# zaphB/freecad.optics_design_workbench

Hardware: AMD Instinct MI355X
Metric: Monte-Carlo rays/sec (whole node), lensesAndMirrors.FCStd (higher is better)
Workload: dtype f64; 1 GPU; benchmark/lensesAndMirrors.FCStd, 1e+08 Monte-Carlo rays per step per GPU (BASELINE configs[2]), Gaussian point source sigma=1e-2, Philox4x32-10 seed 0x0D15EA5E; record_hit_rows=True, histogram=1024x1024 u64, parallelism=ray-index sharding x1, one RCCL reduce

## Files before the change

### freecad/optics_design_workbench_amd/csrc/odw_build.h

```cpp
#pragma once

#include <algorithm>
#include <cmath>
#include <cstdint>
#include <cstdio>
#include <cstring>
#include <limits>
#include <map>
#include <string>
#include <utility>
#include <vector>

namespace {

using namespace odw;

struct HostScene {
  std::vector<double> prim_f64;
  std::vector<int32_t> prim_i32;
  std::vector<int32_t> cond;
  std::vector<double> prim_hdr;
  std::vector<char> dead;
  std::vector<double> group_f64, group_gdir;
  std::vector<int32_t> group_i32;
// ... 1107 lines not shown
    for (std::vector<int>& set : inside[p]) {
      std::sort(set.begin(), set.end());
      set.erase(std::unique(set.begin(), set.end()), set.end());
    }
    std::sort(inside[p].begin(), inside[p].end());
  }
  for (int p = 0; p < n; ++p) {
    box_of[p] = p;
    for (int q = 0; q < p; ++q)
      if (!dead[q] && !dead[p] && hs.prim_i32[4 * q + 1] == hs.prim_i32[4 * p + 1] && inside[q] == inside[p]) {
        box_of[p] = q;
        box_shared[q] = 1;
        break;
      }
  }
}

constexpr int kSpecImageLimits = 4;
constexpr size_t kSpecArgBytes = 4096 - 512;

struct SpecLayout {
  int n = 0, ng = 0, size = 0;
  int gf = 0, gd = 0, gi = 0;
  std::vector<int> frame, par, box, der;
  std::vector<int> box_of, box_shared;
  std::vector<int> dc;
  bool fits(size_t params_bytes) const { return ((params_bytes + 7) & ~(size_t)7) + 8 + (size_t)size * 8 <= kSpecArgBytes; }
};

inline int spec_derived_count(int type) {
  switch (type) {
    case ODW_PRIM_BOX: return 3;
    case ODW_PRIM_CYLINDER: case ODW_PRIM_CONE: case ODW_PRIM_PARABOLOID: case ODW_PRIM_TORUS: return 4;
    case ODW_PRIM_CONICOID: case ODW_PRIM_ASPHERE: return 3;
    default: return 0;
  }
}

inline SpecLayout spec_image_layout(const HostScene& hs, const int32_t* disp_kind = nullptr) {
  SpecLayout L;
  const int n = L.n = hs.n_prims, ng = L.ng = hs.n_groups;
  spec_box_sharing(hs, L.box_of, L.box_shared);
  int at = kSpecImageLimits;
  L.gf = at; at += 4 * ng;
  L.gd = at; at += 3 * ng;
  L.gi = at; at += 2 * ng;
  L.frame.assign(n, 0); L.par.assign(n, 0); L.box.assign(n, -1); L.der.assign(n, -1);
  for (int p = 0; p < n; ++p) {
    const bool faces = (((hs.prim_i32[4 * p + 2]) >> ODW_FACEMASK_SHIFT) & 0xff) != 0;
    L.frame[p] = at; at += __builtin_popcount(xf_stored(xf_pattern(&hs.prim_f64[16 * (size_t)p])));
    L.par[p] = at; at += hs.prim_i32[4 * p] == ODW_PRIM_ASPHERE ? 4 + ODW_ASPH_ROW : 4;
    if (faces && L.box_of[p] == p) { L.box[p] = at; at += 6; }
    const int nd = faces ? spec_derived_count(hs.prim_i32[4 * p]) : 0;
    if (nd) { L.der[p] = at; at += nd; }
  }
  if (disp_kind) {
    L.dc.assign(std::max(1, ng), -1);
    for (int g = 0; g < ng; ++g)
      if (disp_kind[g]) { L.dc[g] = at; at += ODW_DISP_COEFS; }
  }
  L.size = at;
  return L;
}

inline void box_centre_half(double lo, double hi, double& c, double& h) {
#pragma clang fp contract(off)
  c = 0.5 * lo + 0.5 * hi;
  h = std::max(hi - c, c - lo);
  if (!(h >= 0.0)) h = 0.0;
  while (c - h > lo || c + h < hi) h = std::nextafter(h, INFINITY);
}

inline void spec_image_build(const HostScene& hs, const DeviceLimits& lim, const SpecLayout& L, double* img,
                             const double* disp_coef = nullptr) {
#pragma clang fp contract(off)
  const double tol = lim.dist_tol;
  std::fill(img, img + L.size, 0.0);
  if (disp_coef)
    for (int g = 0; g < (int)L.dc.size() && g < L.ng; ++g)
      if (L.dc[g] >= 0) std::memcpy(&img[L.dc[g]], disp_coef + ODW_DISP_COEFS * g, ODW_DISP_COEFS * sizeof(double));
  img[0] = tol;
  img[1] = lim.max_ray_length + tol;
  img[2] = 2.0 * tol;
  for (int g = 0; g < L.ng; ++g) {
    for (int k = 0; k < 4; ++k) img[L.gf + 4 * g + k] = hs.group_f64[4 * (size_t)g + k];
    for (int k = 0; k < 3; ++k) img[L.gd + 3 * g + k] = hs.group_gdir[3 * (size_t)g + k];
    std::memcpy(&img[L.gi + 2 * g], &hs.group_i32[4 * (size_t)g], 4 * sizeof(int32_t));
  }
  for (int p = 0; p < L.n; ++p) {
    const double* pf = &hs.prim_f64[16 * (size_t)p];
    const double* par = pf + 12;
    const unsigned stored = xf_stored(xf_pattern(pf));
    int at = L.frame[p];
    for (int i = 0; i < 12; ++i)
      if ((stored >> i) & 1u) img[at++] = pf[i];
    for (int k = 0; k < 4; ++k) img[L.par[p] + k] = par[k];
    if (hs.prim_i32[4 * p] == ODW_PRIM_ASPHERE)
      for (int k = 0; k < ODW_ASPH_ROW; ++k) img[L.par[p] + 4 + k] = hs.asph[ODW_ASPH_ROW * (size_t)p + k];
    if (L.box[p] >= 0) {
      const double* b = &hs.prim_hdr[8 * (size_t)p];
      for (int a = 0; a < 3; ++a) box_centre_half(b[a], b[3 + a], img[L.box[p] + a], img[L.box[p] + 3 + a]);
    }
    if (L.der[p] < 0) continue;
    double* d = img + L.der[p];
    const int type = hs.prim_i32[4 * p];
    if (type == ODW_PRIM_BOX) {
      for (int a = 0; a < 3; ++a) d[a] = par[a] + tol;
    } else if (type == ODW_PRIM_TORUS) {
      const double R1 = par[0], R2 = par[1];
      d[0] = std::fma(R1 + R2, 1.0000001, 1e-9);
// ... 165 lines not shown
```

### freecad/optics_design_workbench_amd/csrc/odw_capi.hip

```cpp
#include <hip/hip_runtime.h>
#include <hipcub/hipcub.hpp>

#include <algorithm>
#include <atomic>
#include <array>
#include <cmath>
#include <cstdio>
#include <cstdlib>
#include <cstring>
#include <condition_variable>
#include <functional>
#include <mutex>
#include <new>
#include <thread>
#include <string>
#include <utility>
#include <vector>

#include "odw_kernels.hip"
#include "odw_grid.hip"
#include "odw_mesh.hip"
#include "odw_build.h"

using namespace odw;
// ... 1320 lines not shown
int odw_spec_image(const odw_scene_desc* scene, const odw_limits* limits, double* image, uint64_t image_capacity,
                   uint64_t* image_size, int32_t* offsets, uint64_t offsets_capacity, double* boxes,
                   int32_t* in_arguments) {
  if (!scene || !limits) return fail(nullptr, ODW_ERR_INVALID, "odw_spec_image: null argument");
  if (!(limits->dist_tol > 0) || !(limits->max_ray_length > 0)) return fail(nullptr, ODW_ERR_INVALID, "odw_spec_image: limits out of range");
  HostScene tmp;
  std::string refusal;
  int rc = scene_host_tables(scene, tmp, refusal);
  if (rc) return fail(nullptr, rc, refusal);
  std::vector<Box> built;
  compute_boxes(tmp, limits->dist_tol, built);
  const std::string why = spec_ineligible(tmp);
  if (!why.empty()) return fail(nullptr, ODW_ERR_UNSUPPORTED, "odw_spec_image: " + why);
  const SpecLayout L = spec_image_layout(tmp);
  if (image_size) *image_size = (uint64_t)L.size;
  if (in_arguments) *in_arguments = L.fits(sizeof(TraceParams)) ? 1 : 0;
  if (image) {
    if (image_capacity < (uint64_t)L.size) return fail(nullptr, ODW_ERR_CAPACITY, "odw_spec_image: image_capacity too small");
    DeviceLimits lim;
    lim.max_ray_length = limits->max_ray_length;
    lim.dist_tol = limits->dist_tol;
    lim.power_tol = limits->power_tol;
    lim.max_intersections = limits->max_intersections;
    spec_image_build(tmp, lim, L, image);
  }
  if (boxes)
    for (int p = 0; p < L.n; ++p) std::memcpy(boxes + 6 * (size_t)p, &tmp.prim_hdr[8 * (size_t)p], 6 * sizeof(double));
  if (offsets) {
    if (offsets_capacity < 3 + 5 * (uint64_t)L.n) return fail(nullptr, ODW_ERR_CAPACITY, "odw_spec_image: offsets_capacity too small");
    offsets[0] = L.gf; offsets[1] = L.gd; offsets[2] = L.gi;
    for (int p = 0; p < L.n; ++p) {
      int32_t* o = offsets + 3 + 5 * p;
      o[0] = L.frame[p]; o[1] = L.par[p]; o[2] = L.box[p]; o[3] = L.der[p]; o[4] = L.box_of[p];
    }
  }
  return ODW_OK;
}

int odw_build_check(const odw_scene_desc* scene, const odw_limits* limits, int32_t* structure, uint64_t* sizes) {
  if (!scene || !limits) return fail(nullptr, ODW_ERR_INVALID, "odw_build_check: null argument");
  if (!(limits->dist_tol > 0) || limits->max_intersections < 0 || !(limits->max_ray_length > 0))
    return fail(nullptr, ODW_ERR_INVALID, "odw_build_check: limits out of range");
  int flat_limit = kBvhThreshold;
  if (const char* e = getenv("ODW_BVH_THRESHOLD")) flat_limit = atoi(e);
  HostScene tmp;
  SceneAccel A;
  std::string err;
// ... 492 lines not shown
  if (!ctx->have_limits) return fail(ctx, ODW_ERR_NO_SCENE, "odw_upload_scene_batch before odw_set_limits (the boxes carry the tolerance)");
  if (ctx->fresnel_on)
    return fail(ctx, ODW_ERR_UNSUPPORTED, "odw_upload_scene_batch: a batch with a Fresnel mode set (per-scene Fresnel modes are out of scope; "
                                          "odw_set_fresnel with n_groups = 0 clears it)");
  HIPCHK(ctx, hipSetDevice(ctx->device));
  ctx->batch_n = 0;
  ctx->batch_traced = 0;
  ctx->batch_rows_ok = false;
  ctx->phb_valid = ctx->phb_projected = false;
  int rc = odw_upload_scene(ctx, &scenes[0]);
  if (rc) return rc;
  if ((rc = build_bvh(ctx))) return rc;
  const bool compiled = ctx->compile_mode != ODW_COMPILE_OFF && spec_ineligible(ctx->hs).empty();
  const bool rare_compiled = flat_but_for_rare_quadrics(ctx->hs, ctx->flat_limit) && compiled && ctx->compile_mode == ODW_COMPILE_STRUCTURE;
  if ((ctx->P.scene.n_nodes || ctx->P.grid.nx > 0) && !rare_compiled)
    return fail(ctx, ODW_ERR_UNSUPPORTED, "odw_upload_scene_batch: batches are traced by the flat kernels (analytic scenes of up to 64 primitives; "
                                          "with paraboloids, ellipsoids, conicoids or aspheres: by the compiled one, ODW_COMPILE_STRUCTURE)");
  const bool eligible = spec_ineligible(ctx->hs).empty();
  const std::string text0 = eligible ? spec_text(ctx->hs, ctx->n_samplers) : std::string();
  const SpecLayout L0 = eligible ? spec_image_layout(ctx->hs) : SpecLayout();
  bool images = eligible;
  const size_t n = (size_t)ctx->P.scene.n_prims;
  const size_t o_hdr = 16 * n, o_gf = o_hdr + 8 * n, o_gd = o_gf + ODW_MAX_GROUPS * 4, o_img = o_gd + ODW_MAX_GROUPS * 3,
               stride = o_img + (size_t)L0.size;
  std::vector<double> blocks(stride * (size_t)n_scenes, 0.0);
  for (int k = 0; k < n_scenes; ++k) {
    HostScene tmp;
    std::string why;
    if ((rc = scene_host_tables(&scenes[k], tmp, why))) return fail(ctx, rc, why);
    if (!same_structure(ctx->hs, tmp, why))
      return fail(ctx, ODW_ERR_UNSUPPORTED, "odw_upload_scene_batch: scene " + std::to_string(k) + " differs from scene 0 in structure (" + why + ")");
    std::vector<Box> boxes;
    compute_boxes(tmp, ctx->P.lim.dist_tol, boxes);
    if (eligible && spec_text(tmp, ctx->n_samplers) != text0) {
      if (compiled)
        return fail(ctx, ODW_ERR_UNSUPPORTED, "odw_upload_scene_batch: scene " + std::to_string(k) + " differs from scene 0 in the structure a "
                                              "compiled kernel is built from (which frame entries are 0 / +1 / -1, shared boxes)");
      images = false;
    }
    double* b = blocks.data() + stride * (size_t)k;
    if (images) spec_image_build(tmp, ctx->P.lim, L0, b + o_img);
    std::memcpy(b, tmp.prim_f64.data(), 16 * n * sizeof(double));
    std::memcpy(b + o_hdr, tmp.prim_hdr.data(), 8 * n * sizeof(double));
    for (size_t p = 0; p < n; ++p) {
      int32_t w[4];
      std::memcpy(w, b + o_hdr + 8 * p + 6, sizeof w);
      w[2] &= ~ODW_FLAG_ISOLATED;
      std::memcpy(b + o_hdr + 8 * p + 6, w, sizeof w);
    }
    std::memcpy(b + o_gf, tmp.group_f64.data(), ODW_MAX_GROUPS * 4 * sizeof(double));
    std::memcpy(b + o_gd, tmp.group_gdir.data(), ODW_MAX_GROUPS * 3 * sizeof(double));
  }
  if ((rc = upload(ctx, ctx->batch_values, blocks.data(), blocks.size() * sizeof(double)))) return rc;
  std::vector<int32_t> pi = ctx->hs.prim_i32;
  for (size_t p = 0; p < n; ++p) pi[4 * p + 2] &= ~ODW_FLAG_ISOLATED;
  if (n && (rc = upload(ctx, ctx->prim_i32, pi.data(), pi.size() * sizeof(int32_t)))) return rc;
  if ((rc = upload_done(ctx))) return rc;
  ctx->hs.prim_i32 = pi;
  ctx->batch_n = n_scenes;
  ctx->batch_prims = n;
  ctx->batch_stride = stride;
  ctx->batch_img_off = images ? o_img : 0;
  ctx->batch_spec_text = compiled ? text0 : std::string();
  return ODW_OK;
// ... 624 lines not shown
```

### freecad/optics_design_workbench_amd/csrc/odw_kernels.hip

```cpp
#include "odw_device.h"

namespace odw {

#define ODW_CONST __attribute__((address_space(4)))
typedef const double ODW_CONST* cf64;
typedef const int32_t ODW_CONST* ci32;
typedef const uint64_t ODW_CONST* cu64;
template <class T>
__device__ __forceinline__ const T ODW_CONST* as_const(const T* p) {
  return (const T ODW_CONST*)(uintptr_t)p;
}
template <class T>
__device__ __forceinline__ const T* opaque(const T* p) {
  asm volatile("" : "+s"(p));
  return p;
}
typedef const DeviceSource ODW_CONST* csource;
typedef const DeviceDetector ODW_CONST* cdetector;

__device__ __forceinline__ double frcp(double x) {
  double r = __builtin_amdgcn_rcp(x);
  r = fma(fma(-x, r, 1.0), r, r);
  r = fma(fma(-x, r, 1.0), r, r);
  return r;
// ... 114 lines not shown
  return mk(m[0] * p.x + m[1] * p.y + m[2] * p.z + m[3],
            m[4] * p.x + m[5] * p.y + m[6] * p.z + m[7],
            m[8] * p.x + m[9] * p.y + m[10] * p.z + m[11]);
}
template <class P>
__device__ __forceinline__ d3 xf_vec(P m, d3 v) {
  return mk(m[0] * v.x + m[1] * v.y + m[2] * v.z, m[4] * v.x + m[5] * v.y + m[6] * v.z,
            m[8] * v.x + m[9] * v.y + m[10] * v.z);
}
template <class P>
__device__ __forceinline__ d3 xf_vec_t(P m, d3 v) {
  return mk(m[0] * v.x + m[4] * v.y + m[8] * v.z, m[1] * v.x + m[5] * v.y + m[9] * v.z,
            m[2] * v.x + m[6] * v.y + m[10] * v.z);
}

struct NoSpec {
  static constexpr bool enabled = false;
  static constexpr int N = 0;
  static constexpr int NG = 0;
  static constexpr unsigned long long xf(int) { return 0xfffull; }
  static constexpr int type(int) { return 0; }
  static constexpr int gtype(int) { return 0; }
  static constexpr int cond(int) { return 0; }
  static constexpr bool isolated() { return true; }
};
struct NoSource {
  static constexpr bool enabled = false;
  static constexpr bool single_row = false, phi_guide = false, finite_focal = false;
  static constexpr unsigned long long xf = 0xfffull;
};
template <unsigned long long XF, int IA, int IB, int IC, int IT, class P>
__device__ __forceinline__ double xf_comb(P m, double a, double b, double c) {
  double acc = 0.0;
  bool have = false;
#define ODW_XF_TERM(I, V)                                                                            \
  if constexpr (((XF >> (I)) & 1ull) != 0) {                                                         \
    if constexpr (((XF >> (12 + (I))) & 1ull) != 0) acc = have ? acc + (V) : (V);                    \
    else if constexpr (((XF >> (24 + (I))) & 1ull) != 0) acc = have ? acc - (V) : -(V);              \
    else acc = have ? fma(m[I], (V), acc) : m[I] * (V);                                              \
    have = true;                                                                                     \
  }
  ODW_XF_TERM(IB, b)
  ODW_XF_TERM(IA, a)
  ODW_XF_TERM(IC, c)
#undef ODW_XF_TERM
  if constexpr (IT >= 0) {
    if constexpr (((XF >> (IT < 0 ? 0 : IT)) & 1ull) != 0) acc = have ? m[IT < 0 ? 0 : IT] + acc : m[IT < 0 ? 0 : IT];
// ... 845 lines not shown
  a = fma(b.cz, inv.z, -oi.z); w = fabs(inv.z);
  lo = fmax(lo, fma(-b.hz, w, a)); hi = fmin(hi, fma(b.hz, w, a));
  return hi >= fmax(lo, 0.0) && lo < tmax;
}
template <class SPEC>
constexpr bool spec_live(int pi) { return !SPEC::dead(pi) && (SPEC::seq() || ((SPEC::umask() >> SPEC::group(pi)) & 1) != 0); }
template <class SPEC>
constexpr bool spec_own_box(int pi) { return spec_live<SPEC>(pi) && SPEC::box_of(pi) == pi; }
template <class SPEC>
constexpr int spec_next_box(int from) {
  for (int p = from; p < SPEC::N; ++p)
    if (spec_own_box<SPEC>(p)) return p;
  return -1;
}
template <class SPEC, int PI>
__device__ __forceinline__ SpecBox spec_box(const SceneView& sv) {
  static_assert(PI >= 0 && PI < SPEC::N, "box block of a primitive the scene does not have");
  static_assert(SPEC::box(PI) >= 0 && SPEC::box(PI) <= SPEC::IMG - 6, "box block outside the value image");
  cf64 bx = sv.img + SPEC::box(PI);
  return SpecBox{bx[0], bx[1], bx[2], bx[3], bx[4], bx[5]};
}

template <class SPEC, int PI>
__device__ __forceinline__ void spec_prim(const SceneView& sv, Query& q, d3 oi, d3 inv, int skip_solid, int only_solid,
                                          uint64_t mask, bool* boxhit, SpecBox& pending) {
  constexpr int flags = SPEC::flags(PI);
  if constexpr (spec_live<SPEC>(PI)) {
    [[maybe_unused]] const SpecBox own = pending;
    if constexpr (SPEC::box_of(PI) == PI && spec_next_box<SPEC>(PI + 1) >= 0) pending = spec_box<SPEC, spec_next_box<SPEC>(PI + 1)>(sv);
    if ((!SPEC::seq() || ((mask >> SPEC::group(PI)) & 1)) && (flags >> ODW_SOLID_SHIFT) != skip_solid &&
        (!SPEC::isolated() || only_solid < 0 || (flags >> ODW_SOLID_SHIFT) == only_solid)) {
      bool in_box;
      if constexpr (SPEC::box_of(PI) != PI) {
        in_box = boxhit[SPEC::box_of(PI)];
      } else {
        const double cut = q.cut;
        in_box = ray_box_centred(own, oi, inv, cut);
#if ODW_DOUBLE == 1
        in_box = in_box & ray_box_centred(own, mk(opq(oi.x), oi.y, oi.z), inv, cut);
#endif
      }
      boxhit[PI] = in_box;
      if (in_box)
        intersect_prim<SPEC::rare(), SPEC, PI>(sv, q, PI, SPEC::type(PI), SPEC::group(PI), flags, SPEC::cond_word(PI));
#if ODW_DOUBLE == 3 || ODW_DOUBLE == 4 || ODW_DOUBLE == 12
      if (in_box && SPEC::type(PI) == (ODW_DOUBLE == 3 ? ODW_PRIM_CYLINDER : (ODW_DOUBLE == 4 ? ODW_PRIM_BOX : ODW_PRIM_SPHERE))) {
        Query q2 = q;
        q2.start.x = opq(q.start.x);
        intersect_prim<SPEC::rare(), SPEC, PI>(sv, q2, PI, SPEC::type(PI), SPEC::group(PI), flags, SPEC::cond_word(PI));
        q.any = q2.any; q.oth = q2.oth;
      }
#endif
    } else if constexpr (SPEC::box_of(PI) == PI) {
      boxhit[PI] = SPEC::box_shared(PI) ? ray_box_centred(own, oi, inv, q.cut) : false;
    }
  }
}
template <class T, T... I> struct IndexList {};
template <class SPEC, int... PI>
__device__ __forceinline__ void spec_prims(const SceneView& sv, Query& q, d3 oi, d3 inv, int skip_solid, int only_solid,
                                           uint64_t mask, IndexList<int, PI...>) {
  bool boxhit[sizeof...(PI)] = {};
  SpecBox pending = {};
  if constexpr (spec_next_box<SPEC>(0) >= 0) pending = spec_box<SPEC, spec_next_box<SPEC>(0)>(sv);
  (spec_prim<SPEC, PI>(sv, q, oi, inv, skip_solid, only_solid, mask, boxhit, pending), ...);
}

template <bool BVH, class SPEC = NoSpec, bool ASPH = false>
__device__ __forceinline__ int nearest(const DeviceScene& sc, const SceneView& sv,
                                       const DeviceLimits& lim, d3 start, d3 dn, int medium,
                                       uint64_t mask, double& t_hit, int& face,
                                       int* __restrict__ stack, int skip_solid, int only_solid = -1) {
  Query q;
  q.start = start; q.dn = dn;
  if constexpr (SPEC::enabled) { q.tol = sv.lim[0]; q.tmax = sv.lim[1]; }
  else { q.tol = lim.dist_tol; q.tmax = lim.max_ray_length + lim.dist_tol; }
  q.medium = medium;
  q.in_medium = __ballot(medium >= 0) != 0ull;
  q.cut = q.tmax;
  q.any.t = INFINITY; q.any.prim = 0x7fffffff; q.any.face = 0x7fffffff;
  q.oth = q.any;
#if ODW_DOUBLE == 9
  d3 inv = mk(frcp1(dn.x), frcp1(dn.y), frcp1(dn.z));
  d3 oi = mk(start.x * inv.x, start.y * inv.y, start.z * inv.z);
  {
    const d3 dn2 = mk(opq(dn.x), opq(dn.y), opq(dn.z));
    const d3 inv2 = mk(frcp1(dn2.x), frcp1(dn2.y), frcp1(dn2.z));
    const d3 oi2 = mk(start.x * inv2.x, start.y * inv2.y, start.z * inv2.z);
    inv = inv2.x == inv.x ? inv : inv2;
    oi = oi2.y == oi.y ? oi : oi2;
  }
#else
  const d3 inv = mk(frcp1(dn.x), frcp1(dn.y), frcp1(dn.z));
  const d3 oi = mk(start.x * inv.x, start.y * inv.y, start.z * inv.z);
#endif
  if constexpr (SPEC::enabled) {
    spec_prims<SPEC>(sv, q, oi, inv, skip_solid, only_solid, mask, __make_integer_seq<IndexList, int, SPEC::N>{});
  } else if (!BVH) {
    const bool per_lane_mask = sc.seq_enabled != 0;
    const uint64_t umask = sc.all_mask & ~sc.ignore_mask;
    for (int p = 0; p < sc.n_prims; ++p) {
      cf64 hdr = sv.prim_hdr + 8 * p;
      ci32 hi = (ci32)(hdr + 6);
      const int type = hi[0], g = hi[1], flags = hi[2], cond_word = hi[3];
      if (per_lane_mask) {
        if (!((mask >> g) & 1)) continue;
      } else {
        if (!((umask >> g) & 1)) continue;
      }
      if ((flags >> ODW_SOLID_SHIFT) == skip_solid) continue;
      if (only_solid >= 0 && (flags >> ODW_SOLID_SHIFT) != only_solid) continue;
      const double cut = fmin(q.tmax, q.any.t + 2.0 * q.tol);
      if (!ray_box(hdr, oi, inv, cut)) continue;
      intersect_prim<0>(sv, q, p, type, g, flags, cond_word);
    }
  } else {
    typedef const float ODW_CONST* cf32;
    typedef float vf4 __attribute__((ext_vector_type(4)));
    typedef int vi4 __attribute__((ext_vector_type(4)));
    cf32 nodes = (cf32)(uintptr_t)sc.bvh_nodes;
    ci32 bvh_prims = as_const(sc.bvh_prims);
    const float ofx = (float)start.x, ofy = (float)start.y, ofz = (float)start.z;
    const float ivx = (float)inv.x, ivy = (float)inv.y, ivz = (float)inv.z;
    int sp = 0;
    int cur = 0;
    int pend = -1;
    for (;;) {
      for (;;) {
        const unsigned long long looking = __ballot(cur >= 0 && pend == -1);
        if (!(cur >= 0 && (pend == -1 || looking != 0ull))) break;
        cf32 nd = nodes + (size_t)cur * 16;
        const vf4 a0 = *reinterpret_cast<const vf4 ODW_CONST*>(nd);
        const vf4 a1 = *reinterpret_cast<const vf4 ODW_CONST*>(nd + 4);
        const vf4 a2 = *reinterpret_cast<const vf4 ODW_CONST*>(nd + 8);
        const vi4 lk = *reinterpret_cast<const vi4 ODW_CONST*>(nd + 12);
        const float cutf = (float)fmin(q.tmax, q.any.t + 2.0 * q.tol) * 1.00001f + 1e-3f;
        float tn0, tf0, tn1, tf1;
        {
          const float x0 = (a0.x - ofx) * ivx, x1 = (a0.w - ofx) * ivx;
// ... 406 lines not shown
  ray_uniforms(ray, seed, up, ut);
  sample_source(src, up, ut, t, phi);
  make_ray(src, t, phi, r.point, r.dir);
  r.power = src->power;
  return r;
}

template <class SRC>
__device__ __forceinline__ RayInit generate_ray_spec(csource src, uint64_t ray, uint64_t seed) {
  RayInit r;
  double up, ut, t, phi;
  ray_uniforms(ray, seed, up, ut);
  sample_source<true, SRC::phi_guide, SRC::single_row>(src, up, ut, t, phi);
  make_ray<SRC>(src, t, phi, r.point, r.dir);
  r.power = src->power;
  return r;
}

template <class SRC>
__device__ __noinline__ RayInit generate_ray_spec_call(csource src, uint64_t ray, uint64_t seed) {
  return generate_ray_spec<SRC>(src, ray, seed);
}

constexpr bool can_be_medium(int gtype) {
  return gtype != ODW_OPT_MIRROR && gtype != ODW_OPT_ABSORBER && gtype != ODW_OPT_VACUUM;
}
template <class SPEC, int G = 0>
constexpr int spec_media() {
  if constexpr (G >= SPEC::NG) return 0;
  else return (can_be_medium(SPEC::gtype(G)) ? 1 : 0) + spec_media<SPEC, G + 1>();
}
template <class SPEC, int K, int G = 0>
__device__ __forceinline__ double spec_medium_word(cf64 group_f64, int medium, double v) {
  if constexpr (G < SPEC::NG) {
    v = spec_medium_word<SPEC, K, G + 1>(group_f64, medium, v);
    if constexpr (can_be_medium(SPEC::gtype(G))) v = medium == G ? group_f64[4 * G + K] : v;
  }
  return v;
}
template <class SPEC, int K>
__device__ __forceinline__ double medium_word(cf64 group_f64, int medium) {
  if constexpr (SPEC::enabled && spec_media<SPEC>() <= 8) return spec_medium_word<SPEC, K>(group_f64, medium, 0.0);
  else return group_f64[4 * medium + K];
}

template <class SPEC, int G = 0>
__device__ __forceinline__ double spec_chroma_index(cf64 group_f64, int g, double wl, double v) {
  if constexpr (G < SPEC::NG) {
    v = spec_chroma_index<SPEC, G + 1>(group_f64, g, wl, v);
// ... 124 lines not shown
                                         int& skip, int& only, bool& alive, const DeviceChroma* C, double wl) {
  constexpr int flags = SPEC::flags(PI), g = SPEC::group(PI);
  const PackedFrame<SPEC::xf(PI)> pf{sv.img + SPEC::frame(PI)};
  cf64 par = sv.img + SPEC::par(PI);
  d3 n = face_normal<SPEC::rare()>(SPEC::type(PI), par, face, xf_point_nz<SPEC::xf(PI)>(pf, point), par + 4);
  if constexpr ((flags & ODW_FLAG_FLIP_NORMAL) != 0) n = n * -1.0;
  n = xf_vec_t_nz<SPEC::xf(PI)>(pf, n);
#if ODW_DOUBLE == 6
  {
    d3 n2 = face_normal<SPEC::rare()>(SPEC::type(PI), par, face, xf_point_nz<SPEC::xf(PI)>(pf, mk(opq(point.x), point.y, point.z)), par + 4);
    if constexpr ((flags & ODW_FLAG_FLIP_NORMAL) != 0) n2 = n2 * -1.0;
    n2 = xf_vec_t_nz<SPEC::xf(PI)>(pf, n2);
    n = n2.x == n.x ? n : n2;
  }
#endif
  const bool entering = dot(dir, n) < 0;
  if (entering) n = n * -1.0;
  constexpr int fmode = spec_fresnel<SPEC, FRESNEL>(g);
  interact<false, STOCH, LEAN, POWER, SPEC, CHROMA, FRESNEL>(P, group_f64, group_i32, group_gdir, g, SPEC::gtype(g), SPEC::record(g), n, entering, ray,
                               nint, cnt, hit_state, win, point, dir, power, medium, seq, alive, C, wl, fmode);
  const double out = entering ? -dot(dir, n) : dot(dir, n);
  if constexpr ((flags & ODW_FLAG_CONVEX) != 0) skip = out > 0 ? (flags >> ODW_SOLID_SHIFT) : -1;
  else skip = -1;
  if constexpr ((flags & ODW_FLAG_ISOLATED) != 0) only = out < 0 ? (flags >> ODW_SOLID_SHIFT) : -1;
  else only = -1;
}
template <bool STOCH, bool LEAN, bool POWER, class SPEC, bool CHROMA, bool FRESNEL, int... PI>
__device__ __forceinline__ void spec_hits(const TraceParams& P, const SceneView& sv, cf64 group_f64, ci32 group_i32,
                                          cf64 group_gdir, int prim, int face, uint64_t ray, int nint, uint32_t* cnt,
                                          uint32_t* hit_state, uint32_t* win, d3 point, d3& dir, double& power, int& medium, int& seq,
                                          int& skip, int& only, bool& alive, const DeviceChroma* C, double wl, IndexList<int, PI...>) {
  (void)((prim == PI ? (spec_hit<STOCH, LEAN, POWER, SPEC, CHROMA, FRESNEL, PI>(P, sv, group_f64, group_i32, group_gdir, face, ray, nint, cnt, hit_state, win,
                                                  point, dir, power, medium, seq, skip, only, alive, C, wl), true)
                     : false) || ...);
}

__device__ __forceinline__ void close_hit_block(const TraceParams& P, volatile uint32_t* hit_state, uint32_t next_scene) {
  if (!P.out.hit_block) {
    if (P.batch.n_scenes && __lane_id() == 0) hit_state[3] = next_scene;
    return;
  }
  odw_hit* hits = P.out.hits;
  unsigned long long* hit_count = P.out.hit_count;
  if (P.batch.n_scenes) {
    const uint32_t cur = __builtin_amdgcn_readfirstlane(hit_state[3]);
    hits += (size_t)cur * P.out.hit_capacity;
    hit_count += 4 * cur;
// ... 172 lines not shown
          }
#endif
        }
        seq = 0; nint = 0; medium = -1; skip = -1; only = -1;
        alive = true;
        if constexpr (CHROMA)
          wl = C->ray_wl ? C->ray_wl[i] : spectrum_wavelength(C->spec_tab, C->spec_n, C->spec_mode, P.first_ray + i, P.seed);
      }
      next += take;
      if (take == 0 && idle == ~0ull) break;
    }
    ODW_FTIME(0);
    if (alive) {
      if (nint >= lim.max_intersections) {
        ODW_COUNT(ODW_CNT_CAPPED);
        alive = false;
      } else {
      ++nint;
      uint64_t mask = sc.all_mask;
      if (sc.seq_enabled) mask = (seq < sc.seq_len) ? seq_mask[seq] : 0ull;
      mask &= ~sc.ignore_mask;
      double t_hit;
      int face;
      const int prim = nearest<BVH, SPEC, ASPH>(sc, sv, lim, point, dir, medium, mask, t_hit, face,
                                          bvh_stack + threadIdx.x, skip, BVH ? -1 : only);
      if (!BVH && prim < 0 && only >= 0) {
        only = -1;
        --nint;
        continue;
      }
      ODW_FTIME(1);
      if (SEG)
        record_segment(P.out.segs, P.out.seg_capacity, P.out.seg_count, P.first_ray + i, nint - 1, medium, point,
                       point + dir * (prim < 0 ? lim.max_ray_length : t_hit), power);
      if (prim < 0) {
        ODW_COUNT(ODW_CNT_ESCAPED);
        alive = false;
      } else {
      point = point + dir * t_hit;
      if (!LEAN && medium >= 0) {
        const double L = medium_word<SPEC, 2>(group_f64, medium);
        if (L == 0) power = 0;
        else if (L < INFINITY) power = exp(-t_hit / L);
      }
      uint32_t* cnt = cnt_lds + threadIdx.x;
      uint32_t* hit_state = hit_lds + (threadIdx.x >> 6) * 4;
      if constexpr (SPEC::enabled) {
        spec_hits<STOCH, LEAN, POWER, SPEC, CHROMA, FRESNEL>(P, sv, group_f64, group_i32, group_gdir, prim, face, P.first_ray + i, nint, cnt, hit_state,
// ... 350 lines not shown
```

### freecad/optics_design_workbench_amd/csrc/odw_spec.hip

```cpp
#include <dlfcn.h>
#include <hip/hiprtc.h>
#include <sys/stat.h>
#include <unistd.h>

#include <atomic>
#include <chrono>
#include <map>
#include <memory>
#include <mutex>
#include <thread>

#if !defined(__HIP_DEVICE_COMPILE__)
__asm__(
    ".pushsection .rodata\n"
    ".global odw_src_kernels\nodw_src_kernels:\n.incbin \"odw_kernels.hip\"\n.byte 0\n"
    ".global odw_src_device\nodw_src_device:\n.incbin \"odw_device.h\"\n.byte 0\n"
    ".global odw_src_trace\nodw_src_trace:\n.incbin \"../../../include/odw_trace.h\"\n.byte 0\n"
    ".popsection\n");
#endif
extern "C" const char odw_src_kernels[], odw_src_device[], odw_src_trace[];

namespace {

int spec_max_prims() {
// ... 100 lines not shown
    xf[p] = xf_pattern(&hs.prim_f64[16 * (size_t)p]);
  }
  const SpecLayout L = spec_image_layout(hs, disp_kind);
  const std::vector<int>&box_of = L.box_of, &box_shared = L.box_shared;
  std::vector<int> gtype(std::max(1, ng)), grec(std::max(1, ng));
  for (int g = 0; g < ng; ++g) { gtype[g] = hs.group_i32[4 * g]; grec[g] = hs.group_i32[4 * g + 1]; }
  auto fi = [](int v) { return std::to_string(v); };
  auto fu = [](unsigned long long v) { char b[32]; snprintf(b, sizeof b, "0x%llxull", v); return std::string(b); };
  std::string s;
  s += "struct Spec {\n  static constexpr bool enabled = true;\n";
  s += "  static constexpr int N = " + std::to_string(n) + ";\n";
  s += "  static constexpr int NG = " + std::to_string(ng) + ";\n";
  s += table("int", "type", n, type.data(), fi) + table("int", "group", n, group.data(), fi) +
       table("int", "flags", n, flags.data(), fi) + table("int", "cond_word", n, condw.data(), fi) +
       table("bool", "dead", n, dead.data(), fi) + table("int", "box_of", n, box_of.data(), fi) +
       table("bool", "box_shared", n, box_shared.data(), fi) +
       table("int", "cond", (int)hs.cond.size(), hs.cond.data(), fi) +
       table("unsigned long long", "xf", n, xf.data(), fu) + table("int", "gtype", ng, gtype.data(), fi) +
       table("bool", "record", ng, grec.data(), fi);
  int rare = 0;
  for (int p = 0; p < n; ++p) rare |= (type[p] == ODW_PRIM_PARABOLOID ? 1 : 0) | (type[p] == ODW_PRIM_ELLIPSOID ? 2 : 0) | (type[p] == ODW_PRIM_CONICOID ? 4 : 0) |
                                      (type[p] == ODW_PRIM_ASPHERE ? 8 : 0);
  s += "  static constexpr int rare() { return " + std::to_string(rare) + "; }\n";
  s += "  static constexpr bool isolated() { return false; }\n";
  s += "  static constexpr int IMG = " + std::to_string(L.size) + ";\n";
  s += std::string("  static constexpr bool img_fits = ") + (L.fits(sizeof(TraceParams) + (disp_kind ? sizeof(DeviceChroma) : 0)) ? "true" : "false") + ";\n";
  if (disp_kind) {
    std::vector<int> kinds(std::max(1, ng), 0);
    for (int g = 0; g < ng; ++g) kinds[g] = disp_kind[g];
    s += "  static constexpr bool chroma() { return true; }\n";
    s += table("int", "disp", ng, kinds.data(), fi) + table("int", "dc", ng, L.dc.data(), fi);
  }
  bool any_fresnel = false;
  for (int g = 0; fresnel && g < ng; ++g) any_fresnel |= fresnel[g] != 0;
  if (any_fresnel) {
    std::vector<int> modes(std::max(1, ng), 0);
    for (int g = 0; g < ng; ++g) modes[g] = fresnel[g];
    s += table("int", "fresnel", ng, modes.data(), fi);
  }
  s += "  static constexpr int gf = " + std::to_string(L.gf) + ", gd = " + std::to_string(L.gd) + ", gi = " + std::to_string(L.gi) + ";\n";
  s += table("int", "frame", n, L.frame.data(), fi) + table("int", "par", n, L.par.data(), fi) +
       table("int", "box", n, L.box.data(), fi) + table("int", "der", n, L.der.data(), fi);
  s += "  static constexpr int cond_off(int i) { return cond_word(i) & 0xffffff; }\n"
       "  static constexpr int cond_cnt(int i) { return (cond_word(i) >> 24) & 0xff; }\n";
  s += "  static constexpr unsigned long long umask() { return " + fu(hs.all_mask & ~hs.ignore_mask) + "; }\n";
  s += std::string("  static constexpr bool seq() { return ") + (hs.seq_enabled ? "true" : "false") + "; }\n";
  s += "};\n";
  s += std::string("#define ODW_SPEC_LEAN ") + (hs.lean ? "true" : "false") + "\n";
// ... 269 lines not shown
  ctx->spec_fn = it->second.fn;
  ctx->spec_lean = ctx->hs.lean;
  ctx->spec_stoch = ctx->n_samplers > 0;
  return ODW_OK;
}

void spec_note_launch(odw_ctx* ctx, uint64_t n_rays) {
  if (ctx->compile_mode != ODW_COMPILE_AUTO || !ctx->spec_pending) return;
  SpecGlobal& G = spec_global();
  std::lock_guard<std::mutex> lock(G.mu);
  uint64_t& rays = G.rays[ctx->spec_key];
  rays += n_rays;
  if (rays < ctx->spec_hot_rays) return;
  auto jt = G.jobs.find(ctx->spec_key);
  if (jt == G.jobs.end() || jt->second->done.load()) ctx->spec_dirty = true;
}

int spec_launch(odw_ctx* ctx, unsigned grid, hipFunction_t fn, bool batch, const DeviceChroma* chroma = nullptr) {
  const SpecLayout& L = chroma ? ctx->spec_chroma_layout : ctx->spec_layout;
  if (L.n != ctx->hs.n_prims || L.size < kSpecImageLimits) return fail(ctx, ODW_ERR_DEVICE, "compiled kernel without its value image");
  constexpr size_t tail = (sizeof(TraceParams) + 7) & ~(size_t)7;
  const bool resident = !batch && L.fits(sizeof(TraceParams) + (chroma ? sizeof(DeviceChroma) : 0));
  std::vector<double>& img = ctx->spec_image_now;
  img.resize((size_t)L.size);
  spec_image_build(ctx->hs, ctx->P.lim, L, img.data(), chroma ? ctx->disp_coef : nullptr);
  const double* dev = nullptr;
  if (batch) {
    if (!ctx->batch_img_off) return fail(ctx, ODW_ERR_DEVICE, "batch without value images");
    dev = (const double*)ctx->batch_values.p + ctx->batch_img_off;
  } else if (!resident) {
    std::vector<double>& there = ctx->spec_image_host;
    if (there.size() != img.size() || std::memcmp(there.data(), img.data(), img.size() * sizeof(double)) != 0) {
      there.clear();
      int rc = upload(ctx, ctx->spec_image, img.data(), img.size() * sizeof(double));
      if (rc) return rc;
      there = img;
    }
    dev = (const double*)ctx->spec_image.p;
  }
  const size_t nv = resident ? (size_t)L.size : (size_t)kSpecImageLimits;
  std::vector<char>& args = ctx->spec_args;
  static_assert(sizeof(DeviceChroma) % 8 == 0 && alignof(DeviceChroma) == 8, "DeviceChroma follows the tail without padding");
  const size_t tail_end = tail + sizeof(double*) + nv * sizeof(double);
  args.assign(tail_end + (chroma ? sizeof(DeviceChroma) : 0), 0);
  std::memcpy(args.data(), &ctx->P, sizeof(TraceParams));
  std::memcpy(args.data() + tail, &dev, sizeof dev);
  std::memcpy(args.data() + tail + sizeof dev, img.data(), nv * sizeof(double));
  if (chroma) std::memcpy(args.data() + tail_end, chroma, sizeof(DeviceChroma));
  size_t size = args.size();
  void* config[] = {HIP_LAUNCH_PARAM_BUFFER_POINTER, args.data(), HIP_LAUNCH_PARAM_BUFFER_SIZE, &size, HIP_LAUNCH_PARAM_END};
  HIPCHK(ctx, hipModuleLaunchKernel(fn, grid, 1, 1, 256, 1, 1, 0, ctx->stream, nullptr, config));
  return ODW_OK;
}

}
```

Before: 10.40 billion rays/s.

## Add wave-uniform fast path testing only the current isolated solid's primitives

When every lane of a wavefront is inside the same isolated solid (checked with a ballot), the specialized nearest-hit routine intersects only that solid's primitives. It skips the full unrolled scan of all primitives and the ray reciprocal setup. A runtime bitmask of isolated solids is appended to the value image so the compiled kernel can check eligibility, and candidate solids are chosen at compile time. This adds a ballot and readfirstlane per query and slightly enlarges the argument image. Divergent waves fall back to the full scan, and batch launches keep the old path.

```diff
diff --git a/freecad/optics_design_workbench_amd/csrc/odw_build.h b/freecad/optics_design_workbench_amd/csrc/odw_build.h
--- a/freecad/optics_design_workbench_amd/csrc/odw_build.h
+++ b/freecad/optics_design_workbench_amd/csrc/odw_build.h
@@ -1153,10 +1153,12 @@
 struct SpecLayout {
   int n = 0, ng = 0, size = 0;
   int gf = 0, gd = 0, gi = 0;
+  int iso = 0;
   std::vector<int> frame, par, box, der;
   std::vector<int> box_of, box_shared;
   std::vector<int> dc;
-  bool fits(size_t params_bytes) const { return ((params_bytes + 7) & ~(size_t)7) + 8 + (size_t)size * 8 <= kSpecArgBytes; }
+  int words() const { return std::max(size, iso + 1); }
+  bool fits(size_t params_bytes) const { return ((params_bytes + 7) & ~(size_t)7) + 8 + (size_t)words() * 8 <= kSpecArgBytes; }
 };
 
 inline int spec_derived_count(int type) {
@@ -1185,7 +1187,9 @@
     const int nd = faces ? spec_derived_count(hs.prim_i32[4 * p]) : 0;
     if (nd) { L.der[p] = at; at += nd; }
   }
+  L.iso = at;
   if (disp_kind) {
+    at += 1;
     L.dc.assign(std::max(1, ng), -1);
     for (int g = 0; g < ng; ++g)
       if (disp_kind[g]) { L.dc[g] = at; at += ODW_DISP_COEFS; }
@@ -1202,11 +1206,21 @@
   while (c - h > lo || c + h < hi) h = std::nextafter(h, INFINITY);
 }
 
+inline uint64_t spec_isolated_mask(const HostScene& hs) {
+  uint64_t mask = 0;
+  for (int p = 0; p < hs.n_prims; ++p) {
+    const int32_t w = hs.prim_i32[4 * (size_t)p + 2];
+    const int sid = w >> ODW_SOLID_SHIFT;
+    if ((w & ODW_FLAG_ISOLATED) && sid >= 0 && sid < 64) mask |= 1ull << sid;
+  }
+  return mask;
+}
+
 inline void spec_image_build(const HostScene& hs, const DeviceLimits& lim, const SpecLayout& L, double* img,
-                             const double* disp_coef = nullptr) {
+                             const double* disp_coef = nullptr, bool whole = false) {
 #pragma clang fp contract(off)
   const double tol = lim.dist_tol;
-  std::fill(img, img + L.size, 0.0);
+  std::fill(img, img + (whole ? L.words() : L.size), 0.0);
   if (disp_coef)
     for (int g = 0; g < (int)L.dc.size() && g < L.ng; ++g)
       if (L.dc[g] >= 0) std::memcpy(&img[L.dc[g]], disp_coef + ODW_DISP_COEFS * g, ODW_DISP_COEFS * sizeof(double));
@@ -1217,6 +1231,10 @@
     for (int k = 0; k < 4; ++k) img[L.gf + 4 * g + k] = hs.group_f64[4 * (size_t)g + k];
     for (int k = 0; k < 3; ++k) img[L.gd + 3 * g + k] = hs.group_gdir[3 * (size_t)g + k];
     std::memcpy(&img[L.gi + 2 * g], &hs.group_i32[4 * (size_t)g], 4 * sizeof(int32_t));
+  }
+  if (whole) {
+    const uint64_t iso = spec_isolated_mask(hs);
+    std::memcpy(&img[L.iso], &iso, sizeof iso);
   }
   for (int p = 0; p < L.n; ++p) {
     const double* pf = &hs.prim_f64[16 * (size_t)p];
diff --git a/freecad/optics_design_workbench_amd/csrc/odw_capi.hip b/freecad/optics_design_workbench_amd/csrc/odw_capi.hip
--- a/freecad/optics_design_workbench_amd/csrc/odw_capi.hip
+++ b/freecad/optics_design_workbench_amd/csrc/odw_capi.hip
@@ -1366,7 +1366,9 @@
     lim.dist_tol = limits->dist_tol;
     lim.power_tol = limits->power_tol;
     lim.max_intersections = limits->max_intersections;
-    spec_image_build(tmp, lim, L, image);
+    std::vector<double> whole((size_t)L.words());
+    spec_image_build(tmp, lim, L, whole.data(), nullptr, true);
+    std::memcpy(image, whole.data(), (size_t)std::min<uint64_t>(image_capacity, (uint64_t)L.words()) * sizeof(double));
   }
   if (boxes)
     for (int p = 0; p < L.n; ++p) std::memcpy(boxes + 6 * (size_t)p, &tmp.prim_hdr[8 * (size_t)p], 6 * sizeof(double));
@@ -1905,7 +1907,7 @@
   bool images = eligible;
   const size_t n = (size_t)ctx->P.scene.n_prims;
   const size_t o_hdr = 16 * n, o_gf = o_hdr + 8 * n, o_gd = o_gf + ODW_MAX_GROUPS * 4, o_img = o_gd + ODW_MAX_GROUPS * 3,
-               stride = o_img + (size_t)L0.size;
+               stride = o_img + (size_t)(eligible ? L0.words() : 0);
   std::vector<double> blocks(stride * (size_t)n_scenes, 0.0);
   for (int k = 0; k < n_scenes; ++k) {
     HostScene tmp;
@@ -1922,7 +1924,7 @@
       images = false;
     }
     double* b = blocks.data() + stride * (size_t)k;
-    if (images) spec_image_build(tmp, ctx->P.lim, L0, b + o_img);
+    if (images) spec_image_build(tmp, ctx->P.lim, L0, b + o_img, nullptr, true);
     std::memcpy(b, tmp.prim_f64.data(), 16 * n * sizeof(double));
     std::memcpy(b + o_hdr, tmp.prim_hdr.data(), 8 * n * sizeof(double));
     for (size_t p = 0; p < n; ++p) {
diff --git a/freecad/optics_design_workbench_amd/csrc/odw_kernels.hip b/freecad/optics_design_workbench_amd/csrc/odw_kernels.hip
--- a/freecad/optics_design_workbench_amd/csrc/odw_kernels.hip
+++ b/freecad/optics_design_workbench_amd/csrc/odw_kernels.hip
@@ -160,7 +160,6 @@
   static constexpr int type(int) { return 0; }
   static constexpr int gtype(int) { return 0; }
   static constexpr int cond(int) { return 0; }
-  static constexpr bool isolated() { return true; }
 };
 struct NoSource {
   static constexpr bool enabled = false;
@@ -1052,14 +1051,13 @@
 }
 
 template <class SPEC, int PI>
-__device__ __forceinline__ void spec_prim(const SceneView& sv, Query& q, d3 oi, d3 inv, int skip_solid, int only_solid,
+__device__ __forceinline__ void spec_prim(const SceneView& sv, Query& q, d3 oi, d3 inv, int skip_solid,
                                           uint64_t mask, bool* boxhit, SpecBox& pending) {
   constexpr int flags = SPEC::flags(PI);
   if constexpr (spec_live<SPEC>(PI)) {
     [[maybe_unused]] const SpecBox own = pending;
     if constexpr (SPEC::box_of(PI) == PI && spec_next_box<SPEC>(PI + 1) >= 0) pending = spec_box<SPEC, spec_next_box<SPEC>(PI + 1)>(sv);
-    if ((!SPEC::seq() || ((mask >> SPEC::group(PI)) & 1)) && (flags >> ODW_SOLID_SHIFT) != skip_solid &&
-        (!SPEC::isolated() || only_solid < 0 || (flags >> ODW_SOLID_SHIFT) == only_solid)) {
+    if ((!SPEC::seq() || ((mask >> SPEC::group(PI)) & 1)) && (flags >> ODW_SOLID_SHIFT) != skip_solid) {
       bool in_box;
       if constexpr (SPEC::box_of(PI) != PI) {
         in_box = boxhit[SPEC::box_of(PI)];
@@ -1088,19 +1086,89 @@
 }
 template <class T, T... I> struct IndexList {};
 template <class SPEC, int... PI>
-__device__ __forceinline__ void spec_prims(const SceneView& sv, Query& q, d3 oi, d3 inv, int skip_solid, int only_solid,
+__device__ __forceinline__ void spec_prims(const SceneView& sv, Query& q, d3 oi, d3 inv, int skip_solid,
                                            uint64_t mask, IndexList<int, PI...>) {
   bool boxhit[sizeof...(PI)] = {};
   SpecBox pending = {};
   if constexpr (spec_next_box<SPEC>(0) >= 0) pending = spec_box<SPEC, spec_next_box<SPEC>(0)>(sv);
-  (spec_prim<SPEC, PI>(sv, q, oi, inv, skip_solid, only_solid, mask, boxhit, pending), ...);
-}
-
-template <bool BVH, class SPEC = NoSpec, bool ASPH = false>
+  (spec_prim<SPEC, PI>(sv, q, oi, inv, skip_solid, mask, boxhit, pending), ...);
+}
+
+constexpr bool can_be_medium(int gtype) {
+  return gtype != ODW_OPT_MIRROR && gtype != ODW_OPT_ABSORBER && gtype != ODW_OPT_VACUUM;
+}
+template <class SPEC>
+constexpr int spec_solid(int pi) { return SPEC::flags(pi) >> ODW_SOLID_SHIFT; }
+template <class SPEC>
+constexpr int spec_solid_first(int s) {
+  for (int p = 0; p < SPEC::N; ++p)
+    if (spec_live<SPEC>(p) && spec_solid<SPEC>(p) == s) return p;
+  return -1;
+}
+template <class SPEC>
+constexpr bool spec_cand_solid(int s) {
+  if (SPEC::seq() || s < 0 || s >= 64) return false;
+  const int f = spec_solid_first<SPEC>(s);
+  if (f < 0 || !can_be_medium(SPEC::gtype(SPEC::group(f)))) return false;
+  for (int p = f; p < SPEC::N; ++p)
+    if (spec_live<SPEC>(p) && spec_solid<SPEC>(p) == s && SPEC::group(p) != SPEC::group(f)) return false;
+  return true;
+}
+template <class SPEC>
+constexpr int spec_cand_count() {
+  int k = 0;
+  for (int p = 0; p < SPEC::N; ++p)
+    if (spec_live<SPEC>(p) && spec_solid_first<SPEC>(spec_solid<SPEC>(p)) == p && spec_cand_solid<SPEC>(spec_solid<SPEC>(p))) ++k;
+  return k;
+}
+template <class SPEC, int S, int PI>
+__device__ __forceinline__ void spec_solid_prim(const SceneView& sv, Query& q) {
+  if constexpr (spec_live<SPEC>(PI) && spec_solid<SPEC>(PI) == S)
+    intersect_prim<SPEC::rare(), SPEC, PI>(sv, q, PI, SPEC::type(PI), SPEC::group(PI), SPEC::flags(PI), SPEC::cond_word(PI));
+}
+template <class SPEC, int PF, int... PI>
+__device__ __forceinline__ bool spec_uniform_solid(const SceneView& sv, Query& q, int first_only, int only_solid,
+                                                   IndexList<int, PI...>) {
+  constexpr int S = spec_solid<SPEC>(PF);
+  if constexpr (spec_cand_solid<SPEC>(S) && spec_solid_first<SPEC>(S) == PF) {
+    if (first_only == S) {
+      static_assert(SPEC::iso >= 4 && SPEC::iso < SPEC::IMG, "the mask of isolated solids outside the value image");
+      const uint64_t iso = *(cu64)(sv.img + SPEC::iso);
+      const uint64_t others = __ballot(only_solid != S || q.medium != SPEC::group(PF));
+      if (((iso >> S) & 1ull) != 0ull && others == 0ull) {
+        (spec_solid_prim<SPEC, S, PI>(sv, q), ...);
+        return true;
+      }
+    }
+  }
+  return false;
+}
+template <class SPEC, int... PI>
+__device__ __forceinline__ bool spec_uniform(const SceneView& sv, Query& q, int only_solid, IndexList<int, PI...> all) {
+  const int first_only = __builtin_amdgcn_readfirstlane(only_solid);
+  if (first_only < 0) return false;
+  return (spec_uniform_solid<SPEC, PI>(sv, q, first_only, only_solid, all) || ...);
+}
+
+__device__ __forceinline__ void ray_reciprocals(d3 start, d3 dn, d3& inv, d3& oi) {
+  inv = mk(frcp1(dn.x), frcp1(dn.y), frcp1(dn.z));
+  oi = mk(start.x * inv.x, start.y * inv.y, start.z * inv.z);
+#if ODW_DOUBLE == 9
+  {
+    const d3 dn2 = mk(opq(dn.x), opq(dn.y), opq(dn.z));
+    const d3 inv2 = mk(frcp1(dn2.x), frcp1(dn2.y), frcp1(dn2.z));
+    const d3 oi2 = mk(start.x * inv2.x, start.y * inv2.y, start.z * inv2.z);
+    inv = inv2.x == inv.x ? inv : inv2;
+    oi = oi2.y == oi.y ? oi : oi2;
+  }
+#endif
+}
+
+template <bool BVH, class SPEC = NoSpec, bool ASPH = false, bool UNIFORM = true>
 __device__ __forceinline__ int nearest(const DeviceScene& sc, const SceneView& sv,
                                        const DeviceLimits& lim, d3 start, d3 dn, int medium,
                                        uint64_t mask, double& t_hit, int& face,
-                                       int* __restrict__ stack, int skip_solid, int only_solid = -1) {
+                                       int* __restrict__ stack, int skip_solid, int& only_solid) {
   Query q;
   q.start = start; q.dn = dn;
   if constexpr (SPEC::enabled) { q.tol = sv.lim[0]; q.tmax = sv.lim[1]; }
@@ -1110,23 +1178,17 @@
   q.cut = q.tmax;
   q.any.t = INFINITY; q.any.prim = 0x7fffffff; q.any.face = 0x7fffffff;
   q.oth = q.any;
-#if ODW_DOUBLE == 9
-  d3 inv = mk(frcp1(dn.x), frcp1(dn.y), frcp1(dn.z));
-  d3 oi = mk(start.x * inv.x, start.y * inv.y, start.z * inv.z);
-  {
-    const d3 dn2 = mk(opq(dn.x), opq(dn.y), opq(dn.z));
-    const d3 inv2 = mk(frcp1(dn2.x), frcp1(dn2.y), frcp1(dn2.z));
-    const d3 oi2 = mk(start.x * inv2.x, start.y * inv2.y, start.z * inv2.z);
-    inv = inv2.x == inv.x ? inv : inv2;
-    oi = oi2.y == oi.y ? oi : oi2;
-  }
-#else
-  const d3 inv = mk(frcp1(dn.x), frcp1(dn.y), frcp1(dn.z));
-  const d3 oi = mk(start.x * inv.x, start.y * inv.y, start.z * inv.z);
-#endif
+  d3 inv, oi;
   if constexpr (SPEC::enabled) {
-    spec_prims<SPEC>(sv, q, oi, inv, skip_solid, only_solid, mask, __make_integer_seq<IndexList, int, SPEC::N>{});
+    bool uniform = false;
+    if constexpr (UNIFORM && spec_cand_count<SPEC>() > 0) uniform = spec_uniform<SPEC>(sv, q, only_solid, __make_integer_seq<IndexList, int, SPEC::N>{});
+    if (!uniform) {
+      ray_reciprocals(start, dn, inv, oi);
+      spec_prims<SPEC>(sv, q, oi, inv, skip_solid, mask, __make_integer_seq<IndexList, int, SPEC::N>{});
+      only_solid = -1;
+    }
   } else if (!BVH) {
+    ray_reciprocals(start, dn, inv, oi);
     const bool per_lane_mask = sc.seq_enabled != 0;
     const uint64_t umask = sc.all_mask & ~sc.ignore_mask;
     for (int p = 0; p < sc.n_prims; ++p) {
@@ -1145,6 +1207,7 @@
       intersect_prim<0>(sv, q, p, type, g, flags, cond_word);
     }
   } else {
+    ray_reciprocals(start, dn, inv, oi);
     typedef const float ODW_CONST* cf32;
     typedef float vf4 __attribute__((ext_vector_type(4)));
     typedef int vi4 __attribute__((ext_vector_type(4)));
@@ -1597,9 +1660,6 @@
   return generate_ray_spec<SRC>(src, ray, seed);
 }
 
-constexpr bool can_be_medium(int gtype) {
-  return gtype != ODW_OPT_MIRROR && gtype != ODW_OPT_ABSORBER && gtype != ODW_OPT_VACUUM;
-}
 template <class SPEC, int G = 0>
 constexpr int spec_media() {
   if constexpr (G >= SPEC::NG) return 0;
@@ -1770,7 +1830,7 @@
   const double out = entering ? -dot(dir, n) : dot(dir, n);
   if constexpr ((flags & ODW_FLAG_CONVEX) != 0) skip = out > 0 ? (flags >> ODW_SOLID_SHIFT) : -1;
   else skip = -1;
-  if constexpr ((flags & ODW_FLAG_ISOLATED) != 0) only = out < 0 ? (flags >> ODW_SOLID_SHIFT) : -1;
+  if constexpr (spec_cand_solid<SPEC>(flags >> ODW_SOLID_SHIFT)) only = out < 0 ? (flags >> ODW_SOLID_SHIFT) : -1;
   else only = -1;
 }
 template <bool STOCH, bool LEAN, bool POWER, class SPEC, bool CHROMA, bool FRESNEL, int... PI>
@@ -1989,8 +2049,10 @@
       mask &= ~sc.ignore_mask;
       double t_hit;
       int face;
-      const int prim = nearest<BVH, SPEC, ASPH>(sc, sv, lim, point, dir, medium, mask, t_hit, face,
-                                          bvh_stack + threadIdx.x, skip, BVH ? -1 : only);
+      int only_now = BVH ? -1 : only;
+      const int prim = nearest<BVH, SPEC, ASPH, !BATCH>(sc, sv, lim, point, dir, medium, mask, t_hit, face,
+                                          bvh_stack + threadIdx.x, skip, only_now);
+      if constexpr (SPEC::enabled) only = only_now;
       if (!BVH && prim < 0 && only >= 0) {
         only = -1;
         --nint;
diff --git a/freecad/optics_design_workbench_amd/csrc/odw_spec.hip b/freecad/optics_design_workbench_amd/csrc/odw_spec.hip
--- a/freecad/optics_design_workbench_amd/csrc/odw_spec.hip
+++ b/freecad/optics_design_workbench_amd/csrc/odw_spec.hip
@@ -146,8 +146,8 @@
   for (int p = 0; p < n; ++p) rare |= (type[p] == ODW_PRIM_PARABOLOID ? 1 : 0) | (type[p] == ODW_PRIM_ELLIPSOID ? 2 : 0) | (type[p] == ODW_PRIM_CONICOID ? 4 : 0) |
                                       (type[p] == ODW_PRIM_ASPHERE ? 8 : 0);
   s += "  static constexpr int rare() { return " + std::to_string(rare) + "; }\n";
-  s += "  static constexpr bool isolated() { return false; }\n";
-  s += "  static constexpr int IMG = " + std::to_string(L.size) + ";\n";
+  s += "  static constexpr int iso = " + std::to_string(L.iso) + ";\n";
+  s += "  static constexpr int IMG = " + std::to_string(L.words()) + ";\n";
   s += std::string("  static constexpr bool img_fits = ") + (L.fits(sizeof(TraceParams) + (disp_kind ? sizeof(DeviceChroma) : 0)) ? "true" : "false") + ";\n";
   if (disp_kind) {
     std::vector<int> kinds(std::max(1, ng), 0);
@@ -463,8 +463,8 @@
   constexpr size_t tail = (sizeof(TraceParams) + 7) & ~(size_t)7;
   const bool resident = !batch && L.fits(sizeof(TraceParams) + (chroma ? sizeof(DeviceChroma) : 0));
   std::vector<double>& img = ctx->spec_image_now;
-  img.resize((size_t)L.size);
-  spec_image_build(ctx->hs, ctx->P.lim, L, img.data(), chroma ? ctx->disp_coef : nullptr);
+  img.resize((size_t)L.words());
+  spec_image_build(ctx->hs, ctx->P.lim, L, img.data(), chroma ? ctx->disp_coef : nullptr, true);
   const double* dev = nullptr;
   if (batch) {
     if (!ctx->batch_img_off) return fail(ctx, ODW_ERR_DEVICE, "batch without value images");
@@ -479,7 +479,7 @@
     }
     dev = (const double*)ctx->spec_image.p;
   }
-  const size_t nv = resident ? (size_t)L.size : (size_t)kSpecImageLimits;
+  const size_t nv = resident ? (size_t)L.words() : (size_t)kSpecImageLimits;
   std::vector<char>& args = ctx->spec_args;
   static_assert(sizeof(DeviceChroma) % 8 == 0 && alignof(DeviceChroma) == 8, "DeviceChroma follows the tail without padding");
   const size_t tail_end = tail + sizeof(double*) + nv * sizeof(double);
```

Measured after the change: 10.78 billion rays/s (median of 6 runs). 1.04x the previous value.
